# hellovuong/ORB_SLAM3_FAST

Hardware: AMD Instinct MI355X
Metric: ORB extract+match frames/sec @1280×720 stereo (both-eye ORBextractor + ComputeStereoMatches) (higher is better)
Workload: dtype u8; 1 GPU; C3: synthetic 1280x720 rectified stereo pairs, 1500 features, 8 levels, scale 1.2, FAST 20/7, ComputeStereoMatches (bf=0.12*532.03, b=0.12); handles=4, distinct_streams_per_gpu=32, frames_in_ring=3, stereo_matches_pair0=987, parallelism=independent stereo pairs sharded across GPUs, no data-path collective

## Files before the change

include/orbx.h:

```cpp
#ifndef ORBX_H_
#define ORBX_H_

#include <stddef.h>
#include <stdint.h>

#ifdef __cplusplus
extern "C" {
#endif

#define ORBX_MAX_LEVELS 12

#define ORBX_OK 0
#define ORBX_E_EMPTY (-1)
#define ORBX_E_BADARG (-2)
#define ORBX_E_CAPACITY (-3)
#define ORBX_E_HIP (-4)
#define ORBX_E_NODEVICE (-5)
#define ORBX_E_UNSUPPORTED (-6)
#define ORBX_E_TIMEOUT (-7)

typedef struct orbx_keypoint {
  float x, y, size, angle, response;
  int32_t octave, class_id;
} orbx_keypoint;
// ... 568 lines not shown
const char* orbx_stage_name(int stage);
int orbx_level_stats(orbx_extractor* ex, int image, int32_t* w, int32_t* h, int32_t* n_candidates,
                     int32_t* n_selected);


int orbx_clock_probe_start(int device, int spin_us, void** probe);
int orbx_clock_probe_finish(void* probe, double* ghz);

int orbx_copy_probe(int device, size_t bytes, int iters, double* gbps);

void orbx_debug_introsort(uint64_t* v, int n);
int orbx_debug_introsort_device(int device, uint64_t* v, int n);

void orbx_debug_set_detect_list_cap(int cap);
void orbx_debug_set_octree_global(int on);
void orbx_debug_set_stereo_direct(int max_pairs);
int orbx_debug_upload_results(orbx_extractor* ex, int image, const orbx_keypoint* kps, const uint8_t* desc, int n, int mono_index);
void orbx_debug_set_clahe_cell_kernel(int on);
void orbx_debug_set_remap_lds(int on);
int orbx_debug_remap_footprints(const float* map_x, const float* map_y, ptrdiff_t map_stride, int out_w, int out_h, int src_w,
                                int src_h, int n_maps, int32_t* table, int cap, int32_t* tiles_x, int32_t* tiles_y);
int orbx_debug_front_tables(const orbx_params* p, int width, int height, uint32_t* cells, int cells_cap, uint32_t* tiles,
                            int tiles_cap, int32_t info[4]);
int orbx_debug_preproc_plan(const orbx_preproc* pp, int32_t info[8]);
void orbx_debug_set_resize_tail(int first_level, int max_levels, int band_rows);
int orbx_debug_resize_plan(const orbx_extractor* ex, int32_t* first_level, int32_t* n_levels, int32_t* n_bands, int cap);
int orbx_debug_score_map(orbx_extractor* ex, int enable);
int orbx_debug_score_level(orbx_extractor* ex, int image, int level, uint8_t* dst, ptrdiff_t dst_stride);
int orbx_debug_sincos(int device, const float* angles, int n, int fused, float* sin_out, float* cos_out);

#ifdef __cplusplus
}
#endif
#endif
```

orb_slam3_fast_amd/__init__.py:

```python
import ctypes as C
import os

import numpy as np

_HERE = os.path.dirname(os.path.abspath(__file__))
LIB_PATH = os.path.join(_HERE, os.environ.get("ORBX_LIB_NAME", "liborbx.so"))

KP_DTYPE = np.dtype([("x", "<f4"), ("y", "<f4"), ("size", "<f4"), ("angle", "<f4"), ("response", "<f4"),
                     ("octave", "<i4"), ("class_id", "<i4")])
assert KP_DTYPE.itemsize == 28

OK, E_EMPTY, E_BADARG, E_CAPACITY, E_HIP, E_NODEVICE, E_UNSUPPORTED, E_TIMEOUT = 0, -1, -2, -3, -4, -5, -6, -7
TH_HIGH, TH_LOW, HISTO_LENGTH = 100, 50, 30
NUM_STAGES = 8
MP_DTYPE = np.dtype([("proj_x", "<f4"), ("proj_y", "<f4"), ("proj_xr", "<f4"), ("view_cos", "<f4"), ("track_depth", "<f4"),
                     ("predicted_level", "<i4"), ("in_view", "u1"), ("bad", "u1"), ("has_observations", "u1"),
                     ("pad_", "u1"), ("desc", "u1", (32,))])
assert MP_DTYPE.itemsize == 60
PP_DTYPE = np.dtype([("u", "<f4"), ("v", "<f4"), ("ur", "<f4"), ("radius", "<f4"), ("angle", "<f4"), ("min_level", "<i4"),
                     ("max_level", "<i4"), ("valid", "u1"), ("has_observations", "u1"), ("pad_", "u1", (2,)),
                     ("desc", "u1", (32,))])
assert PP_DTYPE.itemsize == 64
FP_DTYPE = np.dtype([("u", "<f4"), ("v", "<f4"), ("ur", "<f4"), ("radius", "<f4"), ("predicted_level", "<i4"), ("valid", "u1"),
                     ("pad_", "u1", (3,)), ("desc", "u1", (32,))])
# ... 162 lines not shown
        L.orbx_profile_enable.argtypes = [vp, i]
        L.orbx_profile_collect.argtypes = [vp, vp, vp]
        L.orbx_stage_name.restype = C.c_char_p
        L.orbx_stage_name.argtypes = [i]
        L.orbx_level_stats.argtypes = [vp, i, vp, vp, vp, vp]
        L.orbx_debug_introsort.argtypes = [vp, i]
        L.orbx_debug_introsort.restype = None
        L.orbx_debug_introsort_device.argtypes = [i, vp, i]
        L.orbx_debug_set_detect_list_cap.argtypes = [i]
        L.orbx_debug_set_detect_list_cap.restype = None
        L.orbx_debug_set_octree_global.argtypes = [i]
        L.orbx_debug_set_octree_global.restype = None
        L.orbx_debug_set_stereo_direct.argtypes = [i]
        L.orbx_debug_set_stereo_direct.restype = None
        L.orbx_debug_set_clahe_cell_kernel.argtypes = [i]
        L.orbx_debug_set_clahe_cell_kernel.restype = None
        L.orbx_debug_upload_results.argtypes = [vp, i, vp, vp, i, i]
        L.orbx_debug_set_remap_lds.argtypes = [i]
        L.orbx_debug_set_remap_lds.restype = None
        L.orbx_debug_remap_footprints.argtypes = [vp, vp, C.c_ssize_t, i, i, i, i, i, vp, i, C.POINTER(i), C.POINTER(i)]
        L.orbx_debug_preproc_plan.argtypes = [vp, vp]
        if hasattr(L, "orbx_debug_front_tables"):
            L.orbx_debug_front_tables.argtypes = [vp, i, i, vp, i, vp, i, vp]
        L.orbx_debug_set_resize_tail.argtypes = [i, i, i]
        L.orbx_debug_set_resize_tail.restype = None
        L.orbx_debug_resize_plan.argtypes = [vp, vp, vp, vp, i]
        L.orbx_debug_sincos.argtypes = [i, vp, i, i, vp, vp]
        L.orbx_debug_score_map.argtypes = [vp, i]
        L.orbx_set_opencv_compat.argtypes = [vp, i]
        L.orbx_debug_score_level.argtypes = [vp, i, i, vp, C.c_ssize_t]
        _lib = L
    return _lib


def _check(rc):
    if rc < 0:
        raise OrbxError(rc, lib().orbx_last_error().decode())
    return rc


def _p(a):
    return a.ctypes.data_as(C.c_void_p)


def device_count():
    return lib().orbx_device_count()
# ... 1074 lines not shown
        raise ValueError("map_x and map_y must be float images of the same size")
    nm, dh, dw = mx.shape
    tx, ty = (dw + 127) // 128, (dh + 7) // 8
    tab = np.zeros((nm, tx, ty, 8), np.int32)
    gx, gy = C.c_int(), C.c_int()
    rc = lib().orbx_debug_remap_footprints(_p(mx), _p(my), dw, dw, dh, src_w, src_h, nm, _p(tab), tab.size, C.byref(gx), C.byref(gy))
    _check(rc)
    if (gx.value, gy.value) != (tx, ty):
        raise OrbxError("unexpected tile grid %d x %d" % (gx.value, gy.value))
    return tab if rc == 1 else None


def front_tables(nfeatures, scaleFactor, nlevels, iniThFAST, minThFAST, width, height):
    prm = _Params(int(nfeatures), float(scaleFactor), int(nlevels), int(iniThFAST), int(minThFAST))
    info = np.zeros(4, np.int32)
    _check(lib().orbx_debug_front_tables(C.byref(prm), width, height, None, 0, None, 0, _p(info)))
    cells = np.zeros((int(info[0]), 16), np.uint32)
    tiles = np.zeros(int(info[1]), np.uint32)
    _check(lib().orbx_debug_front_tables(C.byref(prm), width, height, _p(cells), cells.size, _p(tiles) if tiles.size else None,
                                         tiles.size, _p(info)))
    return cells, tiles, int(info[2]), int(info[3])


class ORBVocabulary:

    def __init__(self, k=None, L=None, parent=None, is_leaf=None, desc=None, weight=None, scoring=0, weighting=0, path=None,
                 device=0):
        h = C.c_void_p()
        if path is not None:
            _check(lib().orbx_vocabulary_load_text(device, path.encode(), C.byref(h)))
        else:
            parent = np.ascontiguousarray(parent, np.int32)
            leaf = np.ascontiguousarray(is_leaf, np.uint8)
            d = np.ascontiguousarray(desc, np.uint8)
            w = np.ascontiguousarray(weight, np.float64)
            _check(lib().orbx_vocabulary_create(device, k, L, scoring, weighting, len(parent), _p(parent), _p(leaf), _p(d), _p(w),
                                                C.byref(h)))
        self._h = h
        info = np.zeros(6, np.int32)
        _check(lib().orbx_vocabulary_info(self._h, _p(info)))
        self.k, self.L, self.n_nodes, self.n_words, self.scoring, self.weighting = (int(x) for x in info)

    def __del__(self):
        if getattr(self, "_h", None):
            lib().orbx_vocabulary_destroy(self._h)
            self._h = None
# ... 483 lines not shown
```

orb_slam3_fast_amd/csrc/orbx_api.hip:

```cpp
#include "orbx_host.h"
#include "orbx_rgbd.h"

namespace orbx_host {
thread_local std::string g_err;
}

namespace {
struct StageTimer {
  orbx_extractor* ex;
  hipStream_t s;
  int stage;
  size_t i0 = 0;
  bool on;
  StageTimer(orbx_extractor* ex_, hipStream_t s_, int stage_)
      : ex(ex_), s(s_), stage(stage_), on(ex_->profiling && (ex_->profStage < 0 || ex_->profStage == stage_)) {
    if (!on) {
      if (s == ex->stream) ex->lastEvValid = false;
      return;
    }
    if (s == ex->stream && ex->lastEvValid) {
      i0 = ex->lastEv;
    } else {
      hipEvent_t e = ex->next_event();
      i0 = ex->evCursor - 1;
// ... 166 lines not shown
        const int cb = (int)xtab[D.xcoef + x0].y;
        const int ce = std::min((int)xtab[D.xcoef + x1].x + 1, S.w - 1);
        const int ndw = ((ce - cb) >> 2) + 1;
        const bool whole = l > 1 || cb + 4 * ndw <= S.w;
        const bool fast = whole && ndw > 64 && ndw <= 85 && nrows <= 24 && rb + 28 <= S.h;
        uint32_t* t = &tab[(size_t)tileOff + 8 * (size_t)(tby * nbx + tbx)];
        t[0] = (uint32_t)(D.xcoef + x0);
        t[1] = (uint32_t)x0 | ((uint32_t)(y1 - y0 + 1) << 16);
        t[2] = (uint32_t)rb | ((uint32_t)nrows << 16);
        t[3] = (uint32_t)cb | ((uint32_t)ndw << 16);
        t[4] = (fast ? kTileFast : 0u) | (whole ? kTileWhole : 0u);
        t[5] = (uint32_t)((long long)y0 * D.pitch);
        t[6] = (uint32_t)tby;
      }
      for (int w = 0; w < 4; w++)
        for (int k = 0; k < 4; k++) {
          const int dy = std::min(y0 + w + 4 * k, D.h - 1);
          const uint32_t sy = yrow[D.ycoef + dy];
          uint32_t* r = &tab[(size_t)rowOff + 16 * (size_t)(4 * tby + w) + 4 * k];
          r[0] = (uint32_t)(uint16_t)yab[2 * (D.ycoef + dy)] | ((uint32_t)(uint16_t)yab[2 * (D.ycoef + dy) + 1] << 16);
          r[1] = (uint32_t)(((int)(sy & 0xFFFFu) - rb) * 512);
          r[2] = (uint32_t)(((int)(sy >> 16) - rb) * 512);
        }
    }
  }
}

void build_cell_records(const Geom& g, std::vector<CellRec>& recs) {
  recs.assign((size_t)g.totalCells, CellRec{});
  const int TPd = g.tileP >> 2;
  for (int l = 0; l < g.nlevels; l++) {
    const LevelDev& L = g.lv[l];
    const int maxBX = L.w - kBorder, maxBY = L.h - kBorder;
    for (int ci = 0; ci < L.nRows; ci++)
      for (int cj = 0; cj < L.nCols; cj++) {
        const int cell = ci * L.nCols + cj;
        CellRec& r = recs[(size_t)L.cellStart + cell];
        const int iniY = kBorder + ci * L.hCell, iniX = kBorder + cj * L.wCell;
        const int maxY = std::min(iniY + L.hCell + 6, maxBY), maxX = std::min(iniX + L.wCell + 6, maxBX);
        const int rw = maxX - iniX, rh = maxY - iniY;
        const int dw = rw - 6, dh = rh - 6;
        r.flags = ((uint32_t)l << 8) | ((uint32_t)L.w << 16) | (l == 0 ? kCellL0 : 0u);
        if (iniY >= maxBY - 3 || iniX >= maxBX - 6 || dw <= 0 || dh <= 0) {
          r.flags |= kCellReject;
          continue;
        }
// ... 208 lines not shown
  if (rc != ORBX_OK) return fail(rc, why);
  const Geom& m = ex->gmax;
  if (g.pyrImg > m.pyrImg || g.candImg > m.candImg || g.selImg > m.selImg || g.cellImg > m.cellImg ||
      g.totalCells > m.totalCells)
    return fail(ORBX_E_CAPACITY, "image within max_width x max_height but its pyramid / cell-grid rounding needs more "
                                 "buffer than the handle's maximum size: create the handle with this size");
  g.outCap = m.outCap;
  g.selImg = m.selImg;
  g.pyrImg = m.pyrImg;
  g.candImg = m.candImg;
  g.cellImg = m.cellImg;
  std::vector<uint4> xtab;
  std::vector<int> yofs;
  std::vector<short> yab;
  build_coefs(g, xtab, yofs, yab);
  HIPC(hipStreamSynchronize(ex->stream));
  HIPC(hipMemcpy(ex->d_xtab.p, xtab.data(), xtab.size() * sizeof(uint4), hipMemcpyHostToDevice));
  HIPC(hipMemcpy(ex->d_yofs.p, yofs.data(), yofs.size() * sizeof(int), hipMemcpyHostToDevice));
  {
    std::vector<uint32_t> yrow, rec;
    build_yrow(g, yofs, yrow);
    HIPC(hipMemcpy(ex->d_yrow.p, yrow.data(), yrow.size() * sizeof(uint32_t), hipMemcpyHostToDevice));
    build_resize_records(g, xtab, yrow, yab, rec);
    if (ex->d_rsRec.n < rec.size()) HIPC(ex->d_rsRec.alloc(rec.size()));
    if (!rec.empty()) HIPC(hipMemcpy(ex->d_rsRec.p, rec.data(), rec.size() * sizeof(uint32_t), hipMemcpyHostToDevice));
  }
  HIPC(hipMemcpy(ex->d_yab.p, yab.data(), yab.size() * sizeof(short), hipMemcpyHostToDevice));
  {
    std::vector<CellRec> recs;
    build_cell_records(g, recs);
    HIPC(hipMemcpy(ex->d_cellRec.p, recs.data(), recs.size() * sizeof(CellRec), hipMemcpyHostToDevice));
  }
  HIPC(prepare_kernels(g));
  std::vector<TailPlan> plans;
  std::vector<TailBand> bands;
  build_tail_plans(g, yofs, plans, bands);
  if (!plans.empty()) {
    if (ex->d_tailBands.n < bands.size()) HIPC(ex->d_tailBands.alloc(bands.size()));
    HIPC(hipMemcpy(ex->d_tailBands.p, bands.data(), bands.size() * sizeof(TailBand), hipMemcpyHostToDevice));
    unsigned lds = 0;
    for (const TailPlan& tp : plans) lds = std::max(lds, tp.ldsBytes);
    HIPC(prepare_resize_tail(lds));
  }
  ex->tails = plans;
  {
    std::vector<TailPlan> lp;
// ... 248 lines not shown
  ok(ex->d_cand.alloc(B * m.candImg));
  ok(ex->d_cellCand.alloc(B * m.cellImg));
  ok(ex->d_cellCount.alloc(B * m.totalCells));
  ok(ex->d_cellPrefix.alloc(B * m.totalCells));
  ok(ex->d_knode.alloc(B * m.candImg));
  ok(ex->d_candCount.alloc(B * m.nlevels));
  ok(ex->d_sel.alloc(B * m.selImg));
  ok(ex->d_selCount.alloc(B * m.nlevels + ORBX_MAX_LEVELS));
  ok(ex->d_slot.alloc(B * m.selImg));
  ok(ex->d_kps.alloc(B * m.outCap));
  ok(ex->d_desc.alloc(B * m.outCap * 32));
  ok(ex->d_nOut.alloc(B));
  ok(ex->d_mono.alloc(B));
  ok(ex->d_lap.alloc(B * 2));
  ok(hipHostMalloc(reinterpret_cast<void**>(&ex->h_lap), (size_t)B * 2 * sizeof(int), hipHostMallocDefault));
  ok(ex->d_xtab.alloc(nx + 64));
  ok(ex->d_cellRec.alloc(m.totalCells));
  {
    int tiles = 0, trows = 0;
    for (int l = 1; l < m.nlevels; l++) {
      tiles += ((m.lv[l].w + 255) / 256 + 1) * ((m.lv[l].h + 15) / 16 + 1);
      trows += (m.lv[l].h + 15) / 16 + 1;
    }
    ok(ex->d_rsRec.alloc((size_t)8 * tiles + 64 * trows + 64));
  }
  ok(ex->d_yofs.alloc(ny + 64));
  ok(ex->d_yrow.alloc(ny + 64));
  ok(ex->d_packCtr.alloc(4));
  if (e == hipSuccess) e = hipMemset(ex->d_packCtr.p, 0, 4 * sizeof(int));
  ok(ex->d_yab.alloc(2 * ny + 64));
  ok(hipHostMalloc(reinterpret_cast<void**>(&ex->hostResults), host_results_bytes(m.outCap), hipHostMallocDefault));
  if (e != hipSuccess) {
    std::string msg = std::string("allocation failed: ") + hipGetErrorString(e);
    orbx_extractor_destroy(ex);
    return fail(ORBX_E_HIP, msg);
  }
  std::memset(ex->hostResults, 0, 64);
  *out = ex;
  return ORBX_OK;
}

void orbx_extractor_destroy(orbx_extractor* ex) {
  if (!ex) return;
  (void)hipSetDevice(ex->device);
  if (ex->stream) (void)hipStreamSynchronize(ex->stream);
  for (auto& e : ex->graphExec) {
    if (e) (void)hipGraphExecDestroy(e);
// ... 636 lines not shown
  const int rc = build_geom(ex.get(), width, height, g, why);
  if (rc != ORBX_OK) return fail(rc, why);
  std::vector<uint4> xtab;
  std::vector<int> yofs;
  std::vector<short> yab;
  std::vector<uint32_t> yrow, rec;
  std::vector<CellRec> cr;
  build_coefs(g, xtab, yofs, yab);
  build_yrow(g, yofs, yrow);
  build_resize_records(g, xtab, yrow, yab, rec);
  build_cell_records(g, cr);
  info[0] = (int32_t)cr.size(); info[1] = (int32_t)rec.size(); info[2] = g.tileP; info[3] = g.tileH;
  if (cells) {
    if (cr.size() * 16 > (size_t)cells_cap) return fail(ORBX_E_CAPACITY, "cell records larger than cells_cap");
    std::memcpy(cells, cr.data(), cr.size() * sizeof(CellRec));
  }
  if (tiles) {
    if (rec.size() > (size_t)tiles_cap) return fail(ORBX_E_CAPACITY, "tile records larger than tiles_cap");
    std::memcpy(tiles, rec.data(), rec.size() * sizeof(uint32_t));
  }
  return ORBX_OK;
}

int orbx_hamming256(const void* a, const void* b) {
  const uint32_t* x = (const uint32_t*)a;
  const uint32_t* y = (const uint32_t*)b;
  int d = 0;
  for (int i = 0; i < 8; i++) d += __builtin_popcount(x[i] ^ y[i]);
  return d;
}

static int enqueue_stereo_match(orbx_extractor* left, int first_left, orbx_extractor* right, int first_right,
                                int n_pairs, float bf, float b, bool withFilter, StereoArgs* argsOut,
                                const ResultPack* packWithBand, bool* packedOut) {
  if (packedOut) *packedOut = false;
  if (!left || !right) return fail(ORBX_E_BADARG, "null handle");
  if (n_pairs <= 0 || first_left < 0 || first_right < 0 || first_left + n_pairs > left->lastN ||
      first_right + n_pairs > right->lastN)
    return fail(ORBX_E_BADARG, "pair range outside the last extraction");
  if (left->device != right->device || left->curW != right->curW || left->curH != right->curH ||
      std::memcmp(&left->prm, &right->prm, sizeof(orbx_params)) != 0)
    return fail(ORBX_E_BADARG, "left and right extractors must share device, image size and parameters");
  if (!(b > 0.f)) return fail(ORBX_E_BADARG, "baseline must be positive");
  HIPC(hipSetDevice(left->device));
  const size_t capL = (size_t)left->gmax.outCap;
  if (left->stereoPairs < n_pairs) {
// ... 347 lines not shown
```

orb_slam3_fast_amd/csrc/orbx_host.h:

```cpp
#ifndef ORBX_HOST_H
#define ORBX_HOST_H
#if defined(__x86_64__) || defined(__i386__)
#include <immintrin.h>
static inline void cpu_pause() { _mm_pause(); }
#else
static inline void cpu_pause() {}
#endif
#include <memory>
#include <new>
#include <chrono>
#include <cmath>
#include <cstdio>
#include <cstdlib>
#include <cstring>
#include <string>
#include <mutex>
#include <vector>

#include "orbx_internal.h"

using namespace orbx;

namespace orbx_host {


extern thread_local std::string g_err;
void build_coefs(const Geom& g, std::vector<uint4>& xtab, std::vector<int>& yofs, std::vector<short>& yab);
void build_cell_records(const Geom& g, std::vector<CellRec>& recs);
void build_yrow(const Geom& g, const std::vector<int>& yofs, std::vector<uint32_t>& yrow);
void build_resize_records(const Geom& g, const std::vector<uint4>& xtab, const std::vector<uint32_t>& yrow, const std::vector<short>& yab,
                          std::vector<uint32_t>& tab);
inline int fail(int code, const std::string& msg) {
  g_err = msg;
  return code;
}
inline double trace_slow_ms() {
  static const double v = getenv("ORBX_TRACE_SLOW") ? atof(getenv("ORBX_TRACE_SLOW")) : 0.0;
  return v;
}
#define HIPC(expr)                                                                                     \
  do {                                                                                                 \
    const double lim_ = trace_slow_ms();                                                               \
    const auto t0_ = lim_ > 0 ? std::chrono::steady_clock::now() : std::chrono::steady_clock::time_point(); \
    hipError_t e_ = (expr);                                                                            \
    if (lim_ > 0) {                                                                                    \
      const double ms_ = std::chrono::duration<double, std::milli>(std::chrono::steady_clock::now() - t0_).count(); \
      if (ms_ > lim_) std::fprintf(stderr, "ORBX_TRACE_SLOW %.2f ms: %s (%s:%d)\n", ms_, #expr, __FILE__, __LINE__); \
    }                                                                                                  \
    if (e_ != hipSuccess)                                                                              \
      return fail(ORBX_E_HIP, std::string(#expr) + ": " + hipGetErrorString(e_));                      \
  } while (0)

inline int cv_round(float v) { return (int)lrintf(v); }
inline int cv_round(double v) { return (int)lrint(v); }
// ... 352 lines not shown
```

orb_slam3_fast_amd/csrc/orbx_internal.h:

```cpp
#pragma once
#include <hip/hip_runtime.h>
#include <stdint.h>
#include <vector>

#include "../../include/orbx.h"

namespace orbx {

constexpr int kEdge = 19;
constexpr int kHalfPatch = 15;
constexpr int kBorder = 16;
constexpr int kMaxIni = 8;

struct LevelDev {
  int w, h, pitch;
  int nCols, nRows, wCell, hCell;
  int cellStart;
  int quota;
  int candCap;
  int cellCap;
  int selOff, selCap;
  int xcoef, ycoef;
  long long off;
  long long candOff;
// ... 72 lines not shown
};
struct TailPlan {
  int lA, nT, nBands, bandOff;
  int tileBytes[2];
  int pitch[ORBX_MAX_LEVELS + 1];
  int rtOff[ORBX_MAX_LEVELS];
  int rtTotal;
  unsigned ldsBytes;
};
hipError_t launch_resize_tail(const Geom& g, const Pyr& p, const TailPlan& tp, const TailBand* bands, int img0, int nimg,
                              const uint4* xtab, const int* yofs, const short* yab, hipStream_t s);
hipError_t prepare_resize_tail(unsigned ldsBytes);
hipError_t raise_dynamic_lds(const void* fn, size_t bytes);

size_t resize_plain_lds(int sw, int sh, int dw, int dh);
hipError_t prepare_resize_plain(int sw, int sh, int dw, int dh);
hipError_t launch_resize_plain(const uint8_t* src, int sw, int sh, long long sp, long long sip, uint8_t* dst, int dw, int dh,
                               long long dp, long long dip, const uint4* xtab, const uint32_t* yrow, const short* yab, int nimg,
                               hipStream_t s);
hipError_t launch_resize(const Geom& g, const Pyr& p, int nimg, int level, const uint4* xtab, const uint32_t* yofs ,
                         const short* yab, const uint32_t* records, hipStream_t s);
int resize_records_layout(const Geom& g, int level, int& tileOff, int& rowOff);
constexpr uint32_t kTileFast = 1u, kTileWhole = 2u;
hipError_t launch_detect(const Geom& g, const Pyr& p, const CellRec* cellRec, int nimg, uint32_t* cellCand, int* cellCount,
                         int level0, int level1, uint8_t* dbgScore, hipStream_t s);
hipError_t launch_octree(const Geom& g, int nimg, const uint32_t* cellCand, const int* cellCount, int* cellPrefix,
                         uint32_t* cand, int* candCount, uint16_t* knode, uint32_t* sel, int* selCount, int level0,
                         int level1, hipStream_t s);
hipError_t launch_blur(const Geom& g, const Pyr& p, int nimg, int level0, int level1, hipStream_t s);
hipError_t launch_slots(const Geom& g, int nimg, const uint32_t* sel, const int* selCount, const int* lap,
                        int* slot, int* nOut, int* mono, hipStream_t s);
hipError_t launch_describe(const Geom& g, const Pyr& p, int nimg, const uint32_t* sel, const int* selCount,
                           const int* slot, orbx_keypoint* kps, uint8_t* desc, int* nOut, int* mono, hipStream_t s);
size_t octree_lds_bytes(const Geom& g);
size_t resize_lds_bytes(const Geom& g);

struct StereoArgs {
  const orbx_keypoint *kL, *kR;
  const uint8_t *dL, *dR;
  const int *nL, *nR;
  int capL, capR;
  int firstL, firstR;
  float bf, b;
  float* uRight;
  float* depth;
  int* sad;
// ... 372 lines not shown
```

orb_slam3_fast_amd/csrc/orbx_kernels.hip:

```cpp
#include <type_traits>
#include <map>
#include <mutex>

#include "orbx_device.h"
#include "orbx_introsort.h"
#include "orbx_sincos.h"
#include "orbx_blur_mfma.h"

namespace orbx {

__constant__ int c_umax[16] = {15, 15, 15, 15, 14, 14, 14, 13, 13, 12, 11, 10, 9, 8, 6, 3};

#define RS_DW 256
#define RS_DR 16
#define RS_HROWS 6
struct ResizeLv {
  struct { int w, h, pitch, xcoef, ycoef; } D;
  struct { int w, h; } S;
  int sp, l;
  int nbx;
  const uint8_t* src; long long srcImg;
  uint8_t* dst; long long dstImg;
  const uint32_t* tiles;
  const uint32_t* rows;
};
constexpr int kResizeXcdRun = 8;
__device__ __forceinline__ uint32_t vblend4(uint2 t0, uint2 t1, uint32_t bb, uint32_t kRound) {
  uint32_t p0, p1, p2, p3, q0, q1, q2, q3, w01, w23;
  asm("v_mad_u32_u16 %0, %1, %2, %3" : "=v"(p0) : "v"(t0.x), "s"(bb), "v"(kRound));
  asm("v_mad_u32_u16 %0, %1, %2, %3 op_sel:[1,0,0,0]" : "=v"(p1) : "v"(t0.x), "s"(bb), "v"(kRound));
  asm("v_mad_u32_u16 %0, %1, %2, %3" : "=v"(p2) : "v"(t0.y), "s"(bb), "v"(kRound));
  asm("v_mad_u32_u16 %0, %1, %2, %3 op_sel:[1,0,0,0]" : "=v"(p3) : "v"(t0.y), "s"(bb), "v"(kRound));
  asm("v_mad_u32_u16 %0, %1, %2, 0 op_sel:[0,1,0,0]" : "=v"(q0) : "v"(t1.x), "s"(bb));
  asm("v_mad_u32_u16 %0, %1, %2, 0 op_sel:[1,1,0,0]" : "=v"(q1) : "v"(t1.x), "s"(bb));
  asm("v_mad_u32_u16 %0, %1, %2, 0 op_sel:[0,1,0,0]" : "=v"(q2) : "v"(t1.y), "s"(bb));
  asm("v_mad_u32_u16 %0, %1, %2, 0 op_sel:[1,1,0,0]" : "=v"(q3) : "v"(t1.y), "s"(bb));
  asm("v_add_u32_sdwa %0, %1, %2 dst_sel:WORD_0 dst_unused:UNUSED_PAD src0_sel:WORD_1 src1_sel:WORD_1" : "=v"(w01) : "v"(p0), "v"(q0));
  asm("v_add_u32_sdwa %0, %1, %2 dst_sel:WORD_1 dst_unused:UNUSED_PRESERVE src0_sel:WORD_1 src1_sel:WORD_1" : "+v"(w01) : "v"(p1), "v"(q1));
  asm("v_add_u32_sdwa %0, %1, %2 dst_sel:WORD_0 dst_unused:UNUSED_PAD src0_sel:WORD_1 src1_sel:WORD_1" : "=v"(w23) : "v"(p2), "v"(q2));
  asm("v_add_u32_sdwa %0, %1, %2 dst_sel:WORD_1 dst_unused:UNUSED_PRESERVE src0_sel:WORD_1 src1_sel:WORD_1" : "+v"(w23) : "v"(p3), "v"(q3));
  asm("v_pk_lshrrev_b16 %0, 2, %1 op_sel_hi:[0,1]" : "=v"(w01) : "v"(w01));
  asm("v_pk_lshrrev_b16 %0, 2, %1 op_sel_hi:[0,1]" : "=v"(w23) : "v"(w23));
  return __builtin_amdgcn_perm(w23, w01, 0x06040200u);
}
template <int NDW, bool TAB>
__global__ __launch_bounds__(256) void k_resize(ResizeLv rl, const uint4* __restrict__ xtab,
                                                const uint32_t* __restrict__ yrow, const short* __restrict__ yab,
                                                int srcRowsMax, int srcDwMaxRt) {
  extern __shared__ __attribute__((aligned(16))) uint8_t smem[];
  const int SDW = NDW ? NDW : srcDwMaxRt;
  const auto D = rl.D;
  const auto S = rl.S;
  const int l = rl.l;
  const int tid = threadIdx.x;
  const int img = blockIdx.z;
  const int tIdx = xcd_run_remap<kResizeXcdRun>((int)blockIdx.x, (int)gridDim.x, (int)blockIdx.z);
  const int sp = rl.sp;
  const uint8_t* src = rl.src + (long long)img * rl.srcImg;
  uint32_t* st = reinterpret_cast<uint32_t*>(smem);
  uint8_t* ht8 = smem + (size_t)srcRowsMax * SDW * 4;
#ifdef RS_PROF
  long long tq0 = wall_clock64();
#endif
  const int qc = tid & 63, w = __builtin_amdgcn_readfirstlane(tid >> 6);
  int x0, rowsHere;
  int rb, nrows, cb, ndw;
  bool whole, fastGeom;
  const uint4* xt;
  uint8_t* dstTile;
  uint32_t vbb[RS_DR / 4];
  int vr0[RS_DR / 4], vr1[RS_DR / 4];
  constexpr int kFastTrips = 8;
  if (TAB) {
    const uint32_t* tr = rl.tiles + 8 * tIdx;
    xt = xtab + tr[0];
    x0 = (int)(tr[1] & 0xFFFFu), rowsHere = (int)(tr[1] >> 16);
    rb = (int)(tr[2] & 0xFFFFu), nrows = (int)(tr[2] >> 16);
    cb = (int)(tr[3] & 0xFFFFu), ndw = (int)(tr[3] >> 16);
    whole = (tr[4] & kTileWhole) != 0, fastGeom = (tr[4] & kTileFast) != 0;
    dstTile = rl.dst + (long long)img * rl.dstImg + tr[5];
    const uint4* rw4 = reinterpret_cast<const uint4*>(rl.rows) + (4 * (int)tr[6] + w) * (RS_DR / 4);
#pragma unroll
    for (int k = 0; k < RS_DR / 4; k++) {
      const uint4 e = rw4[k];
      vbb[k] = e.x, vr0[k] = (int)e.y, vr1[k] = (int)e.z;
    }
  } else {
    const int tby = __builtin_amdgcn_readfirstlane((int)(((float)tIdx + 0.5f) * __builtin_amdgcn_rcpf((float)rl.nbx)));
    const int tbx = tIdx - tby * rl.nbx;
    const int y0 = tby * RS_DR;
    x0 = tbx * RS_DW;
    const int x1 = min(x0 + RS_DW, D.w) - 1, y1 = min(y0 + RS_DR, D.h) - 1;
    rowsHere = y1 - y0 + 1;
    rb = (int)(yrow[D.ycoef + y0] & 0xFFFFu);
    nrows = (int)(yrow[D.ycoef + y1] >> 16) - rb + 1;
    cb = (int)xtab[D.xcoef + x0].y;
    const int ce = min((int)xtab[D.xcoef + x1].x + 1, S.w - 1);
    ndw = ((ce - cb) >> 2) + 1;
    whole = l > 1 || cb + 4 * ndw <= S.w;
    fastGeom = whole && ndw > 64 && ndw <= 85 && nrows <= 3 * kFastTrips && rb + 3 * kFastTrips + 4 <= S.h;
    xt = xtab + D.xcoef + x0;
    dstTile = rl.dst + (long long)img * rl.dstImg + (long long)y0 * D.pitch;
#pragma unroll
    for (int k = 0; k < RS_DR / 4; k++) {
      const int dy = min(y0 + w + 4 * k, D.h - 1);
      const uint32_t sy = yrow[D.ycoef + dy];
      vbb[k] = reinterpret_cast<const uint32_t*>(yab)[D.ycoef + dy];
      vr0[k] = ((int)(sy & 0xFFFFu) - rb) * (RS_DW * 2), vr1[k] = ((int)(sy >> 16) - rb) * (RS_DW * 2);
    }
  }
  uint32_t sel[4], coef[4];
  int ba[4];
#pragma unroll
  for (int j = 0; j < 4; j++) {
    const uint4 e = xt[4 * qc + j];
    ba[j] = (int)e.y - cb;
    sel[j] = e.z;
    coef[j] = e.w;
  }
  {
    if (NDW != 0 && fastGeom) {
      const float inv_nd = __builtin_amdgcn_rcpf((float)ndw);
      const int r0 = (int)(((float)tid + 0.5f) * inv_nd);
      const int c = tid - __mul24(r0, ndw);
      const uint8_t* fb = src + (long long)rb * sp + cb;
      const uint32_t off0 = (uint32_t)(__mul24(r0, sp) + 4 * c);
      uint8_t* sdst = smem + 4 * (__mul24(r0, NDW) + c);
      uint32_t v[kFastTrips];
      const uint8_t* fbk[kFastTrips];
#pragma unroll
      for (int k = 0; k < kFastTrips; k++) fbk[k] = fb + (size_t)(3 * k) * (size_t)sp;
      static_assert(kFastTrips == 8, "the asm below issues eight loads");
      asm volatile(
          "global_load_dword %0, %8, %9\n\t"
          "global_load_dword %1, %8, %10\n\t"
          "global_load_dword %2, %8, %11\n\t"
          "global_load_dword %3, %8, %12\n\t"
          "global_load_dword %4, %8, %13\n\t"
          "global_load_dword %5, %8, %14\n\t"
          "global_load_dword %6, %8, %15\n\t"
          "global_load_dword %7, %8, %16\n\t"
          "s_waitcnt vmcnt(0)"
          : "=&v"(v[0]), "=&v"(v[1]), "=&v"(v[2]), "=&v"(v[3]), "=&v"(v[4]), "=&v"(v[5]), "=&v"(v[6]), "=&v"(v[7])
          : "v"(off0), "s"(fbk[0]), "s"(fbk[1]), "s"(fbk[2]), "s"(fbk[3]), "s"(fbk[4]), "s"(fbk[5]), "s"(fbk[6]), "s"(fbk[7])
          : "memory");
#pragma unroll
      for (int k = 0; k < kFastTrips; k++) *reinterpret_cast<uint32_t*>(sdst + k * (12 * NDW)) = v[k];
    } else
    for (int cbase = 0; cbase < ndw; cbase += 256) {
    const int nd = min(ndw - cbase, 256);
    const float inv_nd = __builtin_amdgcn_rcpf((float)nd);
    const int rpp = __builtin_amdgcn_readfirstlane((int)(256.5f * inv_nd));
    const int r0 = (int)(((float)tid + 0.5f) * inv_nd);
    const int c = cbase + tid - r0 * nd;
    constexpr int kTrips = 8;
    if (whole) {
      const uint8_t* fb = src + (long long)rb * sp + cb;
      const uint32_t offLast = (uint32_t)(__mul24(nrows - 1, sp) + 4 * c), offStep = (uint32_t)(rpp * sp);
      const int idxLast = 4 * (__mul24(nrows - 1, SDW) + c), idxStep = 4 * rpp * SDW;
      for (int rbase = 0; rbase < nrows; rbase += rpp * kTrips) {
        const uint32_t off0 = (uint32_t)(__mul24(rbase + r0, sp) + 4 * c);
        const int idx0 = 4 * (__mul24(rbase + r0, SDW) + c);
        uint32_t v[kTrips];
#pragma unroll
        for (int k = 0; k < kTrips; k++) v[k] = *reinterpret_cast<const uint32_t*>(fb + min(off0 + (uint32_t)k * offStep, offLast));
#pragma unroll
        for (int k = 0; k < kTrips; k++) *reinterpret_cast<uint32_t*>(smem + min(idx0 + k * idxStep, idxLast)) = v[k];
      }
    } else {
      const bool lanes = r0 < rpp;
      const int gx = cb + 4 * c;
      const bool wide = gx + 4 <= S.w;
      for (int rbase = 0; rbase < nrows; rbase += rpp * kTrips) {
        uint32_t v[kTrips];
        const uint8_t* q = src + (long long)(rb + rbase + r0) * sp + gx;
#pragma unroll
        for (int k = 0; k < kTrips; k++) {
          v[k] = 0;
          if (lanes && rbase + r0 + k * rpp < nrows) {
            if (wide) {
              v[k] = *reinterpret_cast<const uint32_t*>(q);
            } else {
              for (int bI = 0; bI < 4; bI++)
                if (gx + bI < S.w) v[k] |= (uint32_t)q[bI] << (8 * bI);
            }
          }
          q += (long long)rpp * sp;
        }
#pragma unroll
        for (int k = 0; k < kTrips; k++)
          if (lanes && rbase + r0 + k * rpp < nrows) st[(rbase + r0 + k * rpp) * SDW + c] = v[k];
      }
    }
    }
  }
#ifdef RS_PROF
  long long tq1 = wall_clock64();
#endif
  __syncthreads();
#ifdef RS_PROF
  long long tq2 = wall_clock64();
#endif
  {
    auto hrow = [&](const uint8_t* rowp, uint8_t* outp) {
      uint32_t t[4];
#pragma unroll
      for (int j = 0; j < 4; j++) {
        const uint32_t* pr = reinterpret_cast<const uint32_t*>(rowp + ba[j]);
        t[j] = udot2_u16(__builtin_amdgcn_perm(pr[1], pr[0], sel[j]), coef[j], 0u);
      }
      uint2 pk;
      pk.x = t[0] >> 4;
      pk.y = t[2] >> 4;
      asm("v_lshrrev_b32_sdwa %0, 4, %1 dst_sel:WORD_1 dst_unused:UNUSED_PRESERVE src0_sel:DWORD src1_sel:DWORD" : "+v"(pk.x) : "v"(t[1]));
      asm("v_lshrrev_b32_sdwa %0, 4, %1 dst_sel:WORD_1 dst_unused:UNUSED_PRESERVE src0_sel:DWORD src1_sel:DWORD" : "+v"(pk.y) : "v"(t[3]));
      *reinterpret_cast<uint2*>(outp) = pk;
    };
    const int rw0 = RS_HROWS * w;
    const uint8_t* rowp = smem + rw0 * SDW * 4;
    uint8_t* outp = ht8 + rw0 * (RS_DW * 2) + 8 * qc;
#pragma unroll
    for (int i = 0; i < RS_HROWS; i++) {
      if (rw0 + i >= nrows) break;
      hrow(rowp + i * SDW * 4, outp + i * (RS_DW * 2));
    }
    for (int r = 4 * RS_HROWS + w; r < nrows; r += 4) hrow(smem + r * SDW * 4, ht8 + r * (RS_DW * 2) + 8 * qc);
  }
#ifdef RS_PROF
  long long tq3 = wall_clock64();
#endif
  __syncthreads();
#ifdef RS_PROF
  long long tq4 = wall_clock64();
#endif
  {
    const int qx = tid & 63;
    const int dx = x0 + 4 * qx;
    uint32_t kRound = 0x20000u;
    asm volatile("" : "+v"(kRound));
    if (dx < D.w) {
// ... 26 lines not shown
  srcDwMax = ((int)((double)RS_DW * S.w / D.w) + 12) / 4 + 1;
  lds = (size_t)srcRowsMax * srcDwMax * 4 + (size_t)srcRowsMax * RS_DW * 2;
}
size_t resize_lds_bytes(const Geom& g) {
  size_t m = 0;
  for (int l = 1; l < g.nlevels; l++) {
    int a, b;
    size_t n;
    resize_footprint(g, l, a, b, n);
    m = n > m ? n : m;
  }
  return m;
}

constexpr int kResizeNdw = 80;
int resize_records_layout(const Geom& g, int level, int& tileOff, int& rowOff) {
  int n = 0;
  tileOff = rowOff = 0;
  for (int l = 1; l < g.nlevels && l <= level; l++) {
    const int nbx = (g.lv[l].w + RS_DW - 1) / RS_DW, nby = (g.lv[l].h + RS_DR - 1) / RS_DR;
    tileOff = n;
    rowOff = n + 8 * nbx * nby;
    n = rowOff + 4 * RS_DR * nby;
  }
  return n;
}

hipError_t launch_resize(const Geom& g, const Pyr& p, int nimg, int level, const uint4* xtab, const uint32_t* yofs,
                         const short* yab, const uint32_t* records, hipStream_t s) {
  const LevelDev& D = g.lv[level];
  int srcRowsMax, srcDwMax;
  size_t lds;
  resize_footprint(g, level, srcRowsMax, srcDwMax, lds);
  const int nbx = (D.w + RS_DW - 1) / RS_DW, nby = (D.h + RS_DR - 1) / RS_DR;
  dim3 grid(nbx * nby, 1, nimg);
  const LevelDev& S = g.lv[level - 1];
  ResizeLv rl;
  rl.nbx = nbx;
  rl.tiles = rl.rows = nullptr;
  if (records) {
    int tileOff, rowOff;
    resize_records_layout(g, level, tileOff, rowOff);
    rl.tiles = records + tileOff;
    rl.rows = records + rowOff;
  }
  rl.D.w = D.w; rl.D.h = D.h; rl.D.pitch = D.pitch; rl.D.xcoef = D.xcoef; rl.D.ycoef = D.ycoef;
  rl.S.w = S.w; rl.S.h = S.h;
  rl.l = level;
  if (level == 1) {
    rl.sp = (int)p.l0Row; rl.src = p.l0; rl.srcImg = p.l0Img;
  } else {
    rl.sp = S.pitch; rl.src = p.pyr + S.off; rl.srcImg = g.pyrImg;
  }
  rl.dst = p.pyr + D.off; rl.dstImg = g.pyrImg;
  auto go = [&](auto kern) { hipLaunchKernelGGL(kern, grid, dim3(256), lds, s, rl, xtab, yofs, yab, srcRowsMax, srcDwMax); };
  if (srcDwMax == kResizeNdw) {
    if (records) go(k_resize<kResizeNdw, true>); else go(k_resize<kResizeNdw, false>);
  } else {
    if (records) go(k_resize<0, true>); else go(k_resize<0, false>);
  }
  return hipGetLastError();
}


static Geom resize_plain_geom(int sw, int sh, int dw, int dh, long long dp, long long dip) {
  Geom g{};
  g.nlevels = 2;
// ... 2140 lines not shown
```

Before: 84150 stereo frames/s.

## Fold narrow right-edge resize tiles into taller strip tiles

For pyramid levels whose last tile column is at most 64 or 128 pixels wide, the resize kernel now merges F vertically adjacent edge tiles into one strip workgroup, so it no longer launches many mostly-idle blocks. Host code builds per-strip records (row coefficients, LDS offsets) appended to the existing record buffer, and the launch shrinks the grid accordingly. The kernel gains a strip path that reuses the shared load and horizontal-filter lambdas, with lanes remapped so that 256 threads cover F times as many rows. This adds a branch and extra table memory, and the gain is confined to edge tiles of the small resize kernels.

```diff
diff --git a/include/orbx.h b/include/orbx.h
--- a/include/orbx.h
+++ b/include/orbx.h
@@ -614,6 +614,7 @@
                                 int src_h, int n_maps, int32_t* table, int cap, int32_t* tiles_x, int32_t* tiles_y);
 int orbx_debug_front_tables(const orbx_params* p, int width, int height, uint32_t* cells, int cells_cap, uint32_t* tiles,
                             int tiles_cap, int32_t info[4]);
+int orbx_debug_strip_tables(const orbx_params* p, int width, int height, uint32_t* strips, int strips_cap, int32_t info[4]);
 int orbx_debug_preproc_plan(const orbx_preproc* pp, int32_t info[8]);
 void orbx_debug_set_resize_tail(int first_level, int max_levels, int band_rows);
 int orbx_debug_resize_plan(const orbx_extractor* ex, int32_t* first_level, int32_t* n_levels, int32_t* n_bands, int cap);
diff --git a/orb_slam3_fast_amd/__init__.py b/orb_slam3_fast_amd/__init__.py
--- a/orb_slam3_fast_amd/__init__.py
+++ b/orb_slam3_fast_amd/__init__.py
@@ -208,6 +208,8 @@
         L.orbx_debug_preproc_plan.argtypes = [vp, vp]
         if hasattr(L, "orbx_debug_front_tables"):
             L.orbx_debug_front_tables.argtypes = [vp, i, i, vp, i, vp, i, vp]
+        if hasattr(L, "orbx_debug_strip_tables"):
+            L.orbx_debug_strip_tables.argtypes = [vp, i, i, vp, i, vp]
         L.orbx_debug_set_resize_tail.argtypes = [i, i, i]
         L.orbx_debug_set_resize_tail.restype = None
         L.orbx_debug_resize_plan.argtypes = [vp, vp, vp, vp, i]
@@ -1328,6 +1330,15 @@
     return cells, tiles, int(info[2]), int(info[3])
 
 
+def strip_tables(nfeatures, scaleFactor, nlevels, iniThFAST, minThFAST, width, height):
+    prm = _Params(int(nfeatures), float(scaleFactor), int(nlevels), int(iniThFAST), int(minThFAST))
+    info = np.zeros(4, np.int32)
+    _check(lib().orbx_debug_strip_tables(C.byref(prm), width, height, None, 0, _p(info)))
+    tab = np.zeros(int(info[0]), np.uint32)
+    _check(lib().orbx_debug_strip_tables(C.byref(prm), width, height, _p(tab) if tab.size else None, tab.size, _p(info)))
+    return tab
+
+
 class ORBVocabulary:
 
     def __init__(self, k=None, L=None, parent=None, is_leaf=None, desc=None, weight=None, scoring=0, weighting=0, path=None,
diff --git a/orb_slam3_fast_amd/csrc/orbx_api.hip b/orb_slam3_fast_amd/csrc/orbx_api.hip
--- a/orb_slam3_fast_amd/csrc/orbx_api.hip
+++ b/orb_slam3_fast_amd/csrc/orbx_api.hip
@@ -212,6 +212,50 @@
           r[1] = (uint32_t)(((int)(sy & 0xFFFFu) - rb) * 512);
           r[2] = (uint32_t)(((int)(sy >> 16) - rb) * 512);
         }
+    }
+  }
+}
+
+void build_resize_strips(const Geom& g, const std::vector<uint4>& xtab, const std::vector<uint32_t>& yrow, const std::vector<short>& yab,
+                         const std::vector<uint32_t>& tab, std::vector<uint32_t>& strips) {
+  ResizeStrips rs;
+  strips.assign((size_t)resize_strips_layout(g, g.nlevels, rs), 0u);
+  for (int l = 1; l < g.nlevels; l++) {
+    const LevelDev &D = g.lv[l], &S = g.lv[l - 1];
+    resize_strips_layout(g, l, rs);
+    uint32_t* dir = &strips[4 * (size_t)(l - 1)];
+    dir[0] = (uint32_t)rs.F, dir[1] = (uint32_t)rs.off, dir[2] = (uint32_t)rs.nFull, dir[3] = (uint32_t)rs.nStrips;
+    if (!rs.F) continue;
+    int tileOff, rowOff;
+    resize_records_layout(g, l, tileOff, rowOff);
+    const int nbx = (D.w + 255) / 256, nby = (D.h + 15) / 16;
+    uint32_t* o = &strips[(size_t)rs.off];
+    for (int tby = 0; tby < nby; tby++)
+      for (int tbx = 0; tbx + 1 < nbx; tbx++, o += 8) std::memcpy(o, &tab[(size_t)tileOff + 8 * (size_t)(tby * nbx + tbx)], 8 * sizeof(uint32_t));
+    const int F = rs.F, SR = 16 * F, hp = 512 / F;
+    const int x0 = (nbx - 1) * 256, x1 = D.w - 1;
+    const int cb = (int)xtab[D.xcoef + x0].y;
+    const int ce = std::min((int)xtab[D.xcoef + x1].x + 1, S.w - 1);
+    const int ndw = ((ce - cb) >> 2) + 1;
+    const bool whole = l > 1 || cb + 4 * ndw <= S.w;
+    for (int sb = 0; sb < rs.nStrips; sb++, o += 8) {
+      const int y0 = sb * SR, y1 = std::min(y0 + SR, D.h) - 1;
+      const int rb = (int)(yrow[D.ycoef + y0] & 0xFFFFu), re = (int)(yrow[D.ycoef + y1] >> 16);
+      o[0] = (uint32_t)(D.xcoef + x0);
+      o[1] = (uint32_t)x0 | ((uint32_t)(y1 - y0 + 1) << 16);
+      o[2] = (uint32_t)rb | ((uint32_t)(re - rb + 1) << 16);
+      o[3] = (uint32_t)cb | ((uint32_t)ndw << 16);
+      o[4] = kTileStrip | (F == 4 ? 2u << 8 : 1u << 8) | (whole ? kTileWhole : 0u);
+      o[5] = (uint32_t)((long long)y0 * D.pitch);
+      o[6] = 0u;
+      o[7] = (uint32_t)(rs.rowOff + 2 * SR * sb);
+      uint32_t* r = &strips[(size_t)rs.off + o[7]];
+      for (int dr = 0; dr < SR; dr++, r += 2) {
+        const int dy = std::min(y0 + dr, D.h - 1);
+        const uint32_t sy = yrow[D.ycoef + dy];
+        r[0] = (uint32_t)(uint16_t)yab[2 * (D.ycoef + dy)] | ((uint32_t)(uint16_t)yab[2 * (D.ycoef + dy) + 1] << 16);
+        r[1] = (uint32_t)(((int)(sy & 0xFFFFu) - rb) * hp) | ((uint32_t)(((int)(sy >> 16) - rb) * hp) << 16);
+      }
     }
   }
 }
@@ -466,6 +510,11 @@
     build_yrow(g, yofs, yrow);
     HIPC(hipMemcpy(ex->d_yrow.p, yrow.data(), yrow.size() * sizeof(uint32_t), hipMemcpyHostToDevice));
     build_resize_records(g, xtab, yrow, yab, rec);
+    {
+      std::vector<uint32_t> strips;
+      build_resize_strips(g, xtab, yrow, yab, rec, strips);
+      rec.insert(rec.end(), strips.begin(), strips.end());
+    }
     if (ex->d_rsRec.n < rec.size()) HIPC(ex->d_rsRec.alloc(rec.size()));
     if (!rec.empty()) HIPC(hipMemcpy(ex->d_rsRec.p, rec.data(), rec.size() * sizeof(uint32_t), hipMemcpyHostToDevice));
   }
@@ -760,7 +809,10 @@
       tiles += ((m.lv[l].w + 255) / 256 + 1) * ((m.lv[l].h + 15) / 16 + 1);
       trows += (m.lv[l].h + 15) / 16 + 1;
     }
-    ok(ex->d_rsRec.alloc((size_t)8 * tiles + 64 * trows + 64));
+    size_t strips = 4 * (size_t)ORBX_MAX_LEVELS;
+    for (int l = 1; l < m.nlevels; l++) strips += 2 * ((size_t)m.lv[l].h + 64 + 16);
+    strips += (size_t)8 * tiles + (size_t)8 * trows;
+    ok(ex->d_rsRec.alloc((size_t)8 * tiles + 64 * trows + 64 + strips));
   }
   ok(ex->d_yofs.alloc(ny + 64));
   ok(ex->d_yrow.alloc(ny + 64));
@@ -1443,6 +1495,35 @@
   return ORBX_OK;
 }
 
+int orbx_debug_strip_tables(const orbx_params* p, int width, int height, uint32_t* strips, int strips_cap, int32_t info[4]) {
+  if (!p || !info || width < 1 || height < 1 || strips_cap < 0 || (strips_cap && !strips) || p->nlevels < 1 ||
+      p->nlevels > ORBX_MAX_LEVELS || p->nfeatures < 1 || !(p->scale_factor > 1.0f))
+    return fail(ORBX_E_BADARG, "bad argument");
+  std::unique_ptr<orbx_extractor> ex(new orbx_extractor());
+  ex->prm = *p;
+  build_tables(ex.get());
+  Geom g;
+  std::string why;
+  const int rc = build_geom(ex.get(), width, height, g, why);
+  if (rc != ORBX_OK) return fail(rc, why);
+  std::vector<uint4> xtab;
+  std::vector<int> yofs;
+  std::vector<short> yab;
+  std::vector<uint32_t> yrow, rec, st;
+  build_coefs(g, xtab, yofs, yab);
+  build_yrow(g, yofs, yrow);
+  build_resize_records(g, xtab, yrow, yab, rec);
+  build_resize_strips(g, xtab, yrow, yab, rec, st);
+  int folded = 0;
+  for (int l = 1; l < g.nlevels; l++) folded += st[4 * (size_t)(l - 1)] != 0;
+  info[0] = (int32_t)st.size(); info[1] = g.nlevels; info[2] = folded; info[3] = (int32_t)rec.size();
+  if (strips) {
+    if (st.size() > (size_t)strips_cap) return fail(ORBX_E_CAPACITY, "strip table larger than strips_cap");
+    std::memcpy(strips, st.data(), st.size() * sizeof(uint32_t));
+  }
+  return ORBX_OK;
+}
+
 int orbx_hamming256(const void* a, const void* b) {
   const uint32_t* x = (const uint32_t*)a;
   const uint32_t* y = (const uint32_t*)b;
diff --git a/orb_slam3_fast_amd/csrc/orbx_host.h b/orb_slam3_fast_amd/csrc/orbx_host.h
--- a/orb_slam3_fast_amd/csrc/orbx_host.h
+++ b/orb_slam3_fast_amd/csrc/orbx_host.h
@@ -30,6 +30,8 @@
 void build_yrow(const Geom& g, const std::vector<int>& yofs, std::vector<uint32_t>& yrow);
 void build_resize_records(const Geom& g, const std::vector<uint4>& xtab, const std::vector<uint32_t>& yrow, const std::vector<short>& yab,
                           std::vector<uint32_t>& tab);
+void build_resize_strips(const Geom& g, const std::vector<uint4>& xtab, const std::vector<uint32_t>& yrow, const std::vector<short>& yab,
+                         const std::vector<uint32_t>& tab, std::vector<uint32_t>& strips);
 inline int fail(int code, const std::string& msg) {
   g_err = msg;
   return code;
diff --git a/orb_slam3_fast_amd/csrc/orbx_internal.h b/orb_slam3_fast_amd/csrc/orbx_internal.h
--- a/orb_slam3_fast_amd/csrc/orbx_internal.h
+++ b/orb_slam3_fast_amd/csrc/orbx_internal.h
@@ -118,6 +118,14 @@
                          const short* yab, const uint32_t* records, hipStream_t s);
 int resize_records_layout(const Geom& g, int level, int& tileOff, int& rowOff);
 constexpr uint32_t kTileFast = 1u, kTileWhole = 2u;
+constexpr uint32_t kTileStrip = 4u;
+struct ResizeStrips {
+  int F;
+  int off;
+  int nFull, nStrips;
+  int rowOff;
+};
+int resize_strips_layout(const Geom& g, int level, ResizeStrips& rs);
 hipError_t launch_detect(const Geom& g, const Pyr& p, const CellRec* cellRec, int nimg, uint32_t* cellCand, int* cellCount,
                          int level0, int level1, uint8_t* dbgScore, hipStream_t s);
 hipError_t launch_octree(const Geom& g, int nimg, const uint32_t* cellCand, const int* cellCount, int* cellPrefix,
diff --git a/orb_slam3_fast_amd/csrc/orbx_kernels.hip b/orb_slam3_fast_amd/csrc/orbx_kernels.hip
--- a/orb_slam3_fast_amd/csrc/orbx_kernels.hip
+++ b/orb_slam3_fast_amd/csrc/orbx_kernels.hip
@@ -43,6 +43,24 @@
   asm("v_pk_lshrrev_b16 %0, 2, %1 op_sel_hi:[0,1]" : "=v"(w23) : "v"(w23));
   return __builtin_amdgcn_perm(w23, w01, 0x06040200u);
 }
+__device__ __forceinline__ uint32_t vblend4v(uint2 t0, uint2 t1, uint32_t bb, uint32_t kRound) {
+  uint32_t p0, p1, p2, p3, q0, q1, q2, q3, w01, w23;
+  asm("v_mad_u32_u16 %0, %1, %2, %3" : "=v"(p0) : "v"(t0.x), "v"(bb), "v"(kRound));
+  asm("v_mad_u32_u16 %0, %1, %2, %3 op_sel:[1,0,0,0]" : "=v"(p1) : "v"(t0.x), "v"(bb), "v"(kRound));
+  asm("v_mad_u32_u16 %0, %1, %2, %3" : "=v"(p2) : "v"(t0.y), "v"(bb), "v"(kRound));
+  asm("v_mad_u32_u16 %0, %1, %2, %3 op_sel:[1,0,0,0]" : "=v"(p3) : "v"(t0.y), "v"(bb), "v"(kRound));
+  asm("v_mad_u32_u16 %0, %1, %2, 0 op_sel:[0,1,0,0]" : "=v"(q0) : "v"(t1.x), "v"(bb));
+  asm("v_mad_u32_u16 %0, %1, %2, 0 op_sel:[1,1,0,0]" : "=v"(q1) : "v"(t1.x), "v"(bb));
+  asm("v_mad_u32_u16 %0, %1, %2, 0 op_sel:[0,1,0,0]" : "=v"(q2) : "v"(t1.y), "v"(bb));
+  asm("v_mad_u32_u16 %0, %1, %2, 0 op_sel:[1,1,0,0]" : "=v"(q3) : "v"(t1.y), "v"(bb));
+  asm("v_add_u32_sdwa %0, %1, %2 dst_sel:WORD_0 dst_unused:UNUSED_PAD src0_sel:WORD_1 src1_sel:WORD_1" : "=v"(w01) : "v"(p0), "v"(q0));
+  asm("v_add_u32_sdwa %0, %1, %2 dst_sel:WORD_1 dst_unused:UNUSED_PRESERVE src0_sel:WORD_1 src1_sel:WORD_1" : "+v"(w01) : "v"(p1), "v"(q1));
+  asm("v_add_u32_sdwa %0, %1, %2 dst_sel:WORD_0 dst_unused:UNUSED_PAD src0_sel:WORD_1 src1_sel:WORD_1" : "=v"(w23) : "v"(p2), "v"(q2));
+  asm("v_add_u32_sdwa %0, %1, %2 dst_sel:WORD_1 dst_unused:UNUSED_PRESERVE src0_sel:WORD_1 src1_sel:WORD_1" : "+v"(w23) : "v"(p3), "v"(q3));
+  asm("v_pk_lshrrev_b16 %0, 2, %1 op_sel_hi:[0,1]" : "=v"(w01) : "v"(w01));
+  asm("v_pk_lshrrev_b16 %0, 2, %1 op_sel_hi:[0,1]" : "=v"(w23) : "v"(w23));
+  return __builtin_amdgcn_perm(w23, w01, 0x06040200u);
+}
 template <int NDW, bool TAB>
 __global__ __launch_bounds__(256) void k_resize(ResizeLv rl, const uint4* __restrict__ xtab,
                                                 const uint32_t* __restrict__ yrow, const short* __restrict__ yab,
@@ -71,8 +89,13 @@
   uint32_t vbb[RS_DR / 4];
   int vr0[RS_DR / 4], vr1[RS_DR / 4];
   constexpr int kFastTrips = 8;
+  bool strip = false;
+  int lgF = 0;
+  const uint2* srow = nullptr;
   if (TAB) {
     const uint32_t* tr = rl.tiles + 8 * tIdx;
+    strip = (tr[4] & kTileStrip) != 0, lgF = (int)((tr[4] >> 8) & 3u);
+    srow = reinterpret_cast<const uint2*>(rl.tiles + tr[7]);
     xt = xtab + tr[0];
     x0 = (int)(tr[1] & 0xFFFFu), rowsHere = (int)(tr[1] >> 16);
     rb = (int)(tr[2] & 0xFFFFu), nrows = (int)(tr[2] >> 16);
@@ -111,12 +134,104 @@
   }
   uint32_t sel[4], coef[4];
   int ba[4];
+  const int ql = TAB ? (qc & (63 >> lgF)) : qc;
 #pragma unroll
   for (int j = 0; j < 4; j++) {
-    const uint4 e = xt[4 * qc + j];
+    const uint4 e = xt[4 * ql + j];
     ba[j] = (int)e.y - cb;
     sel[j] = e.z;
     coef[j] = e.w;
+  }
+  auto hrow = [&](const uint8_t* rowp, uint8_t* outp) {
+    uint32_t t[4];
+#pragma unroll
+    for (int j = 0; j < 4; j++) {
+      const uint32_t* pr = reinterpret_cast<const uint32_t*>(rowp + ba[j]);
+      t[j] = udot2_u16(__builtin_amdgcn_perm(pr[1], pr[0], sel[j]), coef[j], 0u);
+    }
+    uint2 pk;
+    pk.x = t[0] >> 4;
+    pk.y = t[2] >> 4;
+    asm("v_lshrrev_b32_sdwa %0, 4, %1 dst_sel:WORD_1 dst_unused:UNUSED_PRESERVE src0_sel:DWORD src1_sel:DWORD" : "+v"(pk.x) : "v"(t[1]));
+    asm("v_lshrrev_b32_sdwa %0, 4, %1 dst_sel:WORD_1 dst_unused:UNUSED_PRESERVE src0_sel:DWORD src1_sel:DWORD" : "+v"(pk.y) : "v"(t[3]));
+    *reinterpret_cast<uint2*>(outp) = pk;
+  };
+  auto load_general = [&](const int P) {
+    for (int cbase = 0; cbase < ndw; cbase += 256) {
+    const int nd = min(ndw - cbase, 256);
+    const float inv_nd = __builtin_amdgcn_rcpf((float)nd);
+    const int rpp = __builtin_amdgcn_readfirstlane((int)(256.5f * inv_nd));
+    const int r0 = (int)(((float)tid + 0.5f) * inv_nd);
+    const int c = cbase + tid - r0 * nd;
+    constexpr int kTrips = 8;
+    if (whole) {
+      const uint8_t* fb = src + (long long)rb * sp + cb;
+      const uint32_t offLast = (uint32_t)(__mul24(nrows - 1, sp) + 4 * c), offStep = (uint32_t)(rpp * sp);
+      const int idxLast = 4 * (__mul24(nrows - 1, P) + c), idxStep = 4 * rpp * P;
+      for (int rbase = 0; rbase < nrows; rbase += rpp * kTrips) {
+        const uint32_t off0 = (uint32_t)(__mul24(rbase + r0, sp) + 4 * c);
+        const int idx0 = 4 * (__mul24(rbase + r0, P) + c);
+        uint32_t v[kTrips];
+#pragma unroll
+        for (int k = 0; k < kTrips; k++) v[k] = *reinterpret_cast<const uint32_t*>(fb + min(off0 + (uint32_t)k * offStep, offLast));
+#pragma unroll
+        for (int k = 0; k < kTrips; k++) *reinterpret_cast<uint32_t*>(smem + min(idx0 + k * idxStep, idxLast)) = v[k];
+      }
+    } else {
+      const bool lanes = r0 < rpp;
+      const int gx = cb + 4 * c;
+      const bool wide = gx + 4 <= S.w;
+      for (int rbase = 0; rbase < nrows; rbase += rpp * kTrips) {
+        uint32_t v[kTrips];
+        const uint8_t* q = src + (long long)(rb + rbase + r0) * sp + gx;
+#pragma unroll
+        for (int k = 0; k < kTrips; k++) {
+          v[k] = 0;
+          if (lanes && rbase + r0 + k * rpp < nrows) {
+            if (wide) {
+              v[k] = *reinterpret_cast<const uint32_t*>(q);
+            } else {
+              for (int bI = 0; bI < 4; bI++)
+                if (gx + bI < S.w) v[k] |= (uint32_t)q[bI] << (8 * bI);
+            }
+          }
+          q += (long long)rpp * sp;
+        }
+#pragma unroll
+        for (int k = 0; k < kTrips; k++)
+          if (lanes && rbase + r0 + k * rpp < nrows) st[(rbase + r0 + k * rpp) * P + c] = v[k];
+      }
+    }
+    }
+  };
+  if (TAB && strip) {
+    const int F = 1 << lgF, sub = qc >> (6 - lgF);
+    const int dr0 = w * F + sub;
+    uint2 rc[4];
+#pragma unroll
+    for (int k = 0; k < 4; k++) rc[k] = srow[dr0 + 4 * F * k];
+    load_general(ndw);
+    __syncthreads();
+    const int hp = (RS_DW * 2) >> lgF;
+    uint8_t* hts = smem + ((nrows * ndw * 4 + 7) & ~7) + 8 * ql;
+    for (int r = dr0; r < nrows; r += 4 * F) hrow(smem + r * ndw * 4, hts + r * hp);
+    __syncthreads();
+    const int dx = x0 + 4 * ql;
+    uint32_t kRound = 0x20000u;
+    asm volatile("" : "+v"(kRound));
+    if (dx < D.w) {
+#pragma unroll
+      for (int k = 0; k < 4; k++) {
+        const int dr = dr0 + 4 * F * k;
+        if (dr < rowsHere) {
+          const uint2 t0 = *reinterpret_cast<const uint2*>(hts + (rc[k].y & 0xFFFFu));
+          const uint2 t1 = *reinterpret_cast<const uint2*>(hts + (rc[k].y >> 16));
+          const uint32_t outw = vblend4v(t0, t1, rc[k].x, kRound);
+          asm volatile("global_store_dword %0, %1, %2" : : "v"((uint32_t)(__mul24(dr, D.pitch) + dx)), "v"(outw), "s"(dstTile) : "memory");
+        }
+      }
+    }
+    return;
   }
   {
     if (NDW != 0 && fastGeom) {
@@ -147,52 +262,7 @@
 #pragma unroll
       for (int k = 0; k < kFastTrips; k++) *reinterpret_cast<uint32_t*>(sdst + k * (12 * NDW)) = v[k];
     } else
-    for (int cbase = 0; cbase < ndw; cbase += 256) {
-    const int nd = min(ndw - cbase, 256);
-    const float inv_nd = __builtin_amdgcn_rcpf((float)nd);
-    const int rpp = __builtin_amdgcn_readfirstlane((int)(256.5f * inv_nd));
-    const int r0 = (int)(((float)tid + 0.5f) * inv_nd);
-    const int c = cbase + tid - r0 * nd;
-    constexpr int kTrips = 8;
-    if (whole) {
-      const uint8_t* fb = src + (long long)rb * sp + cb;
-      const uint32_t offLast = (uint32_t)(__mul24(nrows - 1, sp) + 4 * c), offStep = (uint32_t)(rpp * sp);
-      const int idxLast = 4 * (__mul24(nrows - 1, SDW) + c), idxStep = 4 * rpp * SDW;
-      for (int rbase = 0; rbase < nrows; rbase += rpp * kTrips) {
-        const uint32_t off0 = (uint32_t)(__mul24(rbase + r0, sp) + 4 * c);
-        const int idx0 = 4 * (__mul24(rbase + r0, SDW) + c);
-        uint32_t v[kTrips];
-#pragma unroll
-        for (int k = 0; k < kTrips; k++) v[k] = *reinterpret_cast<const uint32_t*>(fb + min(off0 + (uint32_t)k * offStep, offLast));
-#pragma unroll
-        for (int k = 0; k < kTrips; k++) *reinterpret_cast<uint32_t*>(smem + min(idx0 + k * idxStep, idxLast)) = v[k];
-      }
-    } else {
-      const bool lanes = r0 < rpp;
-      const int gx = cb + 4 * c;
-      const bool wide = gx + 4 <= S.w;
-      for (int rbase = 0; rbase < nrows; rbase += rpp * kTrips) {
-        uint32_t v[kTrips];
-        const uint8_t* q = src + (long long)(rb + rbase + r0) * sp + gx;
-#pragma unroll
-        for (int k = 0; k < kTrips; k++) {
-          v[k] = 0;
-          if (lanes && rbase + r0 + k * rpp < nrows) {
-            if (wide) {
-              v[k] = *reinterpret_cast<const uint32_t*>(q);
-            } else {
-              for (int bI = 0; bI < 4; bI++)
-                if (gx + bI < S.w) v[k] |= (uint32_t)q[bI] << (8 * bI);
-            }
-          }
-          q += (long long)rpp * sp;
-        }
-#pragma unroll
-        for (int k = 0; k < kTrips; k++)
-          if (lanes && rbase + r0 + k * rpp < nrows) st[(rbase + r0 + k * rpp) * SDW + c] = v[k];
-      }
-    }
-    }
+      load_general(SDW);
   }
 #ifdef RS_PROF
   long long tq1 = wall_clock64();
@@ -202,20 +272,6 @@
   long long tq2 = wall_clock64();
 #endif
   {
-    auto hrow = [&](const uint8_t* rowp, uint8_t* outp) {
-      uint32_t t[4];
-#pragma unroll
-      for (int j = 0; j < 4; j++) {
-        const uint32_t* pr = reinterpret_cast<const uint32_t*>(rowp + ba[j]);
-        t[j] = udot2_u16(__builtin_amdgcn_perm(pr[1], pr[0], sel[j]), coef[j], 0u);
-      }
-      uint2 pk;
-      pk.x = t[0] >> 4;
-      pk.y = t[2] >> 4;
-      asm("v_lshrrev_b32_sdwa %0, 4, %1 dst_sel:WORD_1 dst_unused:UNUSED_PRESERVE src0_sel:DWORD src1_sel:DWORD" : "+v"(pk.x) : "v"(t[1]));
-      asm("v_lshrrev_b32_sdwa %0, 4, %1 dst_sel:WORD_1 dst_unused:UNUSED_PRESERVE src0_sel:DWORD src1_sel:DWORD" : "+v"(pk.y) : "v"(t[3]));
-      *reinterpret_cast<uint2*>(outp) = pk;
-    };
     const int rw0 = RS_HROWS * w;
     const uint8_t* rowp = smem + rw0 * SDW * 4;
     uint8_t* outp = ht8 + rw0 * (RS_DW * 2) + 8 * qc;
@@ -288,6 +344,34 @@
     tileOff = n;
     rowOff = n + 8 * nbx * nby;
     n = rowOff + 4 * RS_DR * nby;
+  }
+  return n;
+}
+
+int resize_strips_layout(const Geom& g, int level, ResizeStrips& rs) {
+  int n = 4 * (g.nlevels - 1);
+  rs = ResizeStrips{};
+  for (int l = 1; l < g.nlevels && l <= level; l++) {
+    const LevelDev &D = g.lv[l], &S = g.lv[l - 1];
+    const int nbx = (D.w + RS_DW - 1) / RS_DW, nby = (D.h + RS_DR - 1) / RS_DR;
+    const int lastW = D.w - (nbx - 1) * RS_DW;
+    int F = lastW <= 64 ? 4 : lastW <= 128 ? 2 : 0;
+    if (F) {
+      int a, b;
+      size_t lds;
+      resize_footprint(g, l, a, b, lds);
+      const size_t rows = (size_t)((double)(RS_DR * F) * S.h / D.h) + 4;
+      const size_t dws = ((size_t)((double)(RS_DW / F) * S.w / D.w) + 12) / 4 + 1;
+      if (((rows * dws * 4 + 7) & ~(size_t)7) + rows * (size_t)(RS_DW * 2 / F) > lds) F = 0;
+    }
+    rs = ResizeStrips{};
+    rs.F = F;
+    rs.off = n;
+    if (!F) continue;
+    rs.nFull = (nbx - 1) * nby;
+    rs.nStrips = (D.h + RS_DR * F - 1) / (RS_DR * F);
+    rs.rowOff = 8 * (rs.nFull + rs.nStrips);
+    n += rs.rowOff + rs.nStrips * RS_DR * F * 2;
   }
   return n;
 }
@@ -309,6 +393,12 @@
     resize_records_layout(g, level, tileOff, rowOff);
     rl.tiles = records + tileOff;
     rl.rows = records + rowOff;
+    ResizeStrips rs;
+    resize_strips_layout(g, level, rs);
+    if (rs.F) {
+      rl.tiles = records + resize_records_layout(g, g.nlevels, tileOff, rowOff) + rs.off;
+      grid.x = (unsigned)(rs.nFull + rs.nStrips);
+    }
   }
   rl.D.w = D.w; rl.D.h = D.h; rl.D.pitch = D.pitch; rl.D.xcoef = D.xcoef; rl.D.ycoef = D.ycoef;
   rl.S.w = S.w; rl.S.h = S.h;
```

Measured after the change: 84120 stereo frames/s. Within noise of the previous version (-0.0%).
